# pyMSE/NLOTrajectories

Hardware: AMD Instinct MI355X
Metric: solved trajectories/sec (50-knot unicycle+learned-SDF) (higher is better)
Workload: dtype f64 (interior-point solver) + f32 (SDF-MLP: fp32-equivalent split-bf16 MFMA products, as the reference's fp32 libtorch graph)

## Files before the change

nlotrajectories_amd/csrc/nlot_solver.hip:

```cpp
#include <hip/hip_runtime.h>

#include <algorithm>
#include <chrono>
#include <type_traits>
#include <cmath>
#include <cstdlib>
#include <cstdio>
#include <cstring>
#include <vector>

#include "nlot_device.h"
#include "nlot_internal.h"
#include "nlot_solver_ws.h"

namespace nlot {

#ifndef NLOT_WPE_A
#define NLOT_WPE_A 2
#endif
#ifndef NLOT_WPE_B
#define NLOT_WPE_B 2
#endif
#ifndef NLOT_WPE_ACC
#define NLOT_WPE_ACC 3
// ... 2350 lines not shown
            const double dy = AT(X, (seg + 1) * NX + 1) - AT(X, seg * NX + 1);
            const double rr = sqrt(dx * dx + dy * dy + p.path_eps);
            const double sgn = seg == k ? -1.0 : 1.0;
            r[0] += sgn * dx / rr;
            r[1] += sgn * dy / rr;
        }
        if (k > 0)
#pragma unroll
            for (int i = 0; i < NX; ++i) r[i] += AT(yk, (k - 1) * NX + i);
        double A[NX][NX], Bu[NX][NU];
        if (k < N) {
            double x[NX], u[NU];
#pragma unroll
            for (int i = 0; i < NX; ++i) x[i] = AT(X, k * NX + i);
#pragma unroll
            for (int i = 0; i < NU; ++i) u[i] = AT(U, k * NU + i);
            Dyn<DYN>::jac(x, u, p.dt, p.wheelbase, A, Bu);
#pragma unroll
            for (int j = 0; j < NX; ++j) {
                double t = 0;
#pragma unroll
                for (int i = 0; i < NX; ++i) t += A[i][j] * AT(yk, k * NX + i);
                r[j] -= t;
            }
        }
        if (k == 0)
#pragma unroll
            for (int i = 0; i < NX; ++i) r[i] += AT(yi, i);
        if (k == N)
#pragma unroll
            for (int i = 0; i < NX; ++i)
                for (int cc = 0; cc < nc; ++cc)
                    if (dm.tidx[cc] == i) r[i] += AT(yt, cc);
        for (int j = 0; j < M; ++j)
            for (int a = 0; a < 3 && a < NX; ++a) r[a] += AT(Jd, (k * M + j) * 3 + a) * AT(yd, k * M + j);
#pragma unroll
        for (int i = 0; i < NX; ++i) {
            dual = fmax(dual, fabs(r[i]));
            dsq += r[i] * r[i];
            d1 += fabs(r[i]);
        }
        if (k < N)
#pragma unroll
            for (int i = 0; i < NU; ++i) {
                double t = dm.gcb ? AT(yb, k * NU + i) : -AT(zl, k * NU + i) + AT(zu, k * NU + i);
                if (p.use_smooth && k < N - 1) t += 2.0 * p.smooth_weight * AT(U, k * NU + i);
#pragma unroll
                for (int a = 0; a < NX; ++a) t -= Bu[a][i] * AT(yk, k * NX + a);
                dual = fmax(dual, fabs(t));
                dsq += t * t;
                d1 += fabs(t);
            }
        if (dm.ns) {
            double t = 2.0 * p.slack_penalty * AT(S, k) + (dm.gcb ? AT(yb, N * NU + k) : -AT(zs, k));
            if (dm.sd)
                for (int j = 0; j < M; ++j) t += AT(yd, k * M + j);
            dual = fmax(dual, fabs(t));
            dsq += t * t;
            d1 += fabs(t);
        }
        for (int j = 0; j < M; ++j) {
            const double t = -AT(yd, k * M + j) - AT(vt, k * M + j);
            dual = fmax(dual, fabs(t));
            dsq += t * t;
            d1 += fabs(t);
        }
    }
    p_bs.run(ngb, lane, ld_bs, [&](int q, const double* v) {
        const double t = q < nnu ? -v[0] - v[1] + v[2] : -v[0] - v[1];
        dual = fmax(dual, fabs(t));
        dsq += t * t;
        d1 += fabs(t);
    });
    auto pri_ = [&](double v) {
        primal = fmax(primal, fabs(v));
        psq += v * v;
        p1 += fabs(v);
    };
    auto pri1 = [&](int, const double* v) { pri_(v[0]); };
    p_rci.run(NX, lane, ld_rci, pri1);
    p_rct.run(nc, lane, ld_rct, pri1);
    p_rcd.run(N * NX, lane, ld_rcd, pri1);
    cviol = wmax(primal);
    p_rcq.run((N + 1) * M, lane, ld_rcq, [&](int, const double* v) {
        pri_(v[0]);
        cviol = fmax(cviol, fmax(0.0, -v[1]));
    });
    p_rcb.run(ngb, lane, ld_rcb, [&](int q, const double* v) {
        pri_(v[0]);
        if (q < nnu) {
            const double u = v[1];
            cviol = fmax(cviol, fmax(0.0, fmax(p.umin[q % NU] - u, u - p.umax[q % NU])));
        } else {
            cviol = fmax(cviol, fmax(0.0, -v[1]));
        }
    });
    auto compl_ = [&](double z, double s) {
        c0 = fmax(c0, fabs(z * s));
        cmu = fmax(cmu, fabs(z * s - mu0));
        csum += z * s;
        zsum += fabs(z);
        nzc += 1;
    };
    p_cu.run(N * NU, lane, ld_cu, [&](int e, const double* v) {
        compl_(v[1], v[0] - p.umin[e % NU]);
        compl_(v[2], p.umax[e % NU] - v[0]);
    });
    auto compl2 = [&](int, const double* v) { compl_(v[0], v[1]); };
    if (dm.ns) p_zs.run(N + 1, lane, ld_zs, compl2);
    p_vt.run((N + 1) * M, lane, ld_vt, compl2);
    auto ysum1 = [&](int, const double* v) { ysum += fabs(v[0]); };
    p_yi.run(NX, lane, ld_yi, ysum1);
    p_yk.run(N * NX, lane, ld_yk, ysum1);
    p_yt.run(nc, lane, ld_yt, ysum1);
    p_yd.run((N + 1) * M, lane, ld_yd, ysum1);
    p_yb.run(ngb, lane, ld_yb, ysum1);
    dual = wmax(dual);
    primal = wmax(primal);
    cviol = wmax(cviol);
    c0 = wmax(c0);
    cmu = wmax(cmu);
    zsum = wsum(zsum);
    ysum = wsum(ysum);
    nzc = wsum(nzc);
    const double csum_w = wsum(csum), dsq_w = wsum(dsq), psq_w = wsum(psq);
    const double d1_w = wsum(d1), p1_w = wsum(p1);
    const double ny = NX + N * NX + nc + (N + 1) * M + ngb;
    const double sd = fmax(100.0, (ysum + zsum) / (ny + nzc)) / 100.0;
    const double scc = fmax(100.0, zsum / nzc) / 100.0;
    const double E0 = fmax(fmax(dual / sd, primal), c0 / scc);
    KPROF(0, 3);
    const double n_pd = (double)((N + 1) * NX + N * NU + dm.ns * (N + 1) + (N + 1) * M + ngb) +
                        (double)(NX + nc + N * NX + (N + 1) * M + ngb) + nzc;
    auto pd_error = [&](double m) {
        double c1 = 0;
        for (int e = lane; e < N * NU; e += 64) {
            const double u = BVU(e);
            c1 += fabs(AT(zl, e) * (u - p.umin[e % NU]) - m) + fabs(AT(zu, e) * (p.umax[e % NU] - u) - m);
        }
        if (dm.ns)
            for (int k = lane; k <= N; k += 64) c1 += fabs(AT(zs, k) * BVS(k) - m);
        for (int q = lane; q < (N + 1) * M; q += 64) c1 += fabs(AT(vt, q) * AT(T, q) - m);
        return (d1_w + p1_w + wsum(c1)) / n_pd;
    };
    if (ph == PH_SOFT2) {
        const double pd_t = pd_error(SC(SC_MUPD));
        const bool ok = isfinite(pd_t) && pd_t <= o.soft_resto_pderror_reduction_factor * SC(SC_PDC);
        wsync();
        if (!ok) {
            double* buf = &AT(sts, 0);
            iter_io(ws, b, lane, buf, false);
            wsync();
            resto_enter(o, p, dm, ws, b, lane, cnt_next);
            return;
        }
        if (lane == 0) {
            SC(SC_ITERS) = SC(SC_ITERS) + 1;
            SC(SC_INSOFT) = 1;
            SC(SC_TINYLAST) = 0;
            SC(SC_PHASE) = PH_EVAL;
        }
        wsync();
    }
    const int iters = (int)SC(SC_ITERS);
    wsync();
    auto finish = [&](int status) {
        if (lane == 0) {
            SC(SC_E0) = E0;
            SC(SC_STATUS) = status;
            SC(SC_PHASE) = PH_DONE;
        }
    };
    if (!isfinite(E0)) return finish(NLOT_NUMERIC);
    if (E0 <= o.tol && dual <= o.dual_inf_tol && cviol <= o.constr_viol_tol && c0 <= o.compl_inf_tol)
        return finish(NLOT_SOLVED);
    if (iters >= o.max_iter) return finish(NLOT_MAXITER);
    const double kap = o.barrier_tol_factor;
    const double mu_floor = fmin(o.tol, o.compl_inf_tol) / (kap + 1.0);
    constexpr double kMuMin = 1e-11;
    double mu = mu0, tau = SC(SC_TAU);
    bool reset_filter = false;
    auto compl_mu = [&](double m) {
        double cm = 0;
        chunked_update<4, 3>(N * NU, lane, [&](int e, double* v) { v[0] = BVU(e); v[1] = AT(zl, e); v[2] = AT(zu, e); },
                             [&](int e, const double* v) {
                                 cm = fmax(cm, fabs(v[1] * (v[0] - p.umin[e % NU]) - m));
                                 cm = fmax(cm, fabs(v[2] * (p.umax[e % NU] - v[0]) - m));
                             });
        auto cm2 = [&](int, const double* v) { cm = fmax(cm, fabs(v[0] * v[1] - m)); };
        if (dm.ns) chunked_update<4, 2>(N + 1, lane, [&](int k, double* v) { v[0] = AT(zs, k); v[1] = BVS(k); }, cm2);
        chunked_update<4, 2>((N + 1) * M, lane, [&](int q, double* v) { v[0] = AT(vt, q); v[1] = AT(T, q); }, cm2);
        return wmax(cm);
    };
    bool tiny_last = o.mu_strategy == 0 && SC(SC_TINYLAST) != 0.0;
    auto barrier_decrease = [&](double cm) {
        for (;;) {
            const double Emu = fmax(fmax(dual / sd, primal), cm / scc);
            if (Emu > kap * mu && !tiny_last) break;
            tiny_last = false;
            const double nm = fmax(fmin(0.2 * mu, pow(mu, 1.5)), mu_floor);
            if (nm >= mu) break;
            mu = nm;
            tau = fmax(0.99, 1.0 - mu);
            reset_filter = true;
            cm = compl_mu(mu);
        }
    };
    bool use_qf = false;
    const double avg = csum_w / nzc;
    if (o.mu_strategy == 0) {
        if (iters > 0) barrier_decrease(cmu);
    } else {
        double mu_max = SC(SC_MUMAX);
        bool free_ = SC(SC_FREE) != 0.0;
        int naf = (int)SC(SC_NAF);
        if (iters == 0) {
            mu_max = 1e3 * avg;
            free_ = true;
            naf = 0;
        }
        double th_c, ph_c, f_c;
        theta_phi(mu0, &th_c, &ph_c, &f_c);
        auto af_ok = [&]() {
            const double m = 1e-5 * fmin(1.0, th_c);
            bool bad = false;
            for (int i = lane; i < naf; i += 64)
                if (f_c + m >= AT(afilt, 2 * i) && th_c + m >= AT(afilt, 2 * i + 1)) bad = true;
            return __ballot(bad) == 0ull;
        };
        if (!free_) {
            if (af_ok()) {
                free_ = true;
            } else if (fmax(fmax(dual / sd, primal), cmu / scc) <= kap * mu) {
                const double nm = fmax(fmin(0.2 * mu, pow(mu, 1.5)), mu_floor);
                if (nm < mu) {
                    mu = nm;
                    tau = fmax(0.99, 1.0 - mu);
                    reset_filter = true;
                }
            }
        }
        int naf_new = naf;
        if (free_) {
            if (af_ok()) {
                const double m = 1e-5 * fmin(1.0, th_c), nf = f_c - m, nt = th_c - m;
                wsync();
                if (lane == 0) SC(SC_NAF) = naf;
                wsync();
                naf_new = filter_update(ws, b, &AT(afilt, 0), SC_NAF, nf, nt, cnt, lane);
            } else {
                free_ = false;
                mu = fmin(fmax(0.8 * avg, kMuMin), mu_max);
                tau = fmax(0.99, 1.0 - mu);
                reset_filter = true;
            }
        }
        if (lane == 0) {
            SC(SC_NAF) = naf_new;
            SC(SC_FREE) = free_ ? 1.0 : 0.0;
            SC(SC_MUMAX) = mu_max;
        }
        use_qf = free_;
    }
    const double mu_pd = (o.mu_strategy == 1 && use_qf) ? 0.0 : mu;
    const double pd_c = pd_error(mu_pd);
    wsync();
    if (lane == 0) {
        SC(SC_MU) = mu;
        SC(SC_TAU) = tau;
        if (reset_filter) {
            SC(SC_NFILT) = 0;
            SC(SC_INSOFT) = 0;
            SC(SC_SOFTCNT) = 0;
            SC(SC_WD) = 0;
            SC(SC_WDSHORT) = 0;
        }
        SC(SC_PDC) = pd_c;
        SC(SC_MUPD) = mu_pd;
    }
    wsync();
    KPROF(0, 4);
    SV::template build_stages<false>(p, dm, ws, b, lane, MODE_NEWTON, 0.0, use_qf ? 0.0 : mu, avg, use_qf ? 2 : 1, SL);
    KPROF(0, 5);
    KPROF_COUNT(0);
    if (lane == 0) {
        SC(SC_E0) = E0;
        SC(SC_RMU0) = use_qf ? 0.0 : mu;
        SC(SC_RMU1) = avg;
        SC(SC_RNR) = use_qf ? 2 : 1;
        SC(SC_USEQF) = use_qf ? 1.0 : 0.0;
        SC(SC_AVG) = avg;
        SC(SC_DSQ) = dsq_w;
        SC(SC_PSQ) = psq_w;
        SC(SC_NZC) = nzc;
        SC(SC_PRIMAL) = primal;
        SC(SC_RICFIX) = -1.0;
        SC(SC_RIC) = 1;
        ws.ricl[atomicAdd(&cnt[4], 1)] = b;
    }
}

template <int DYN>
__global__ __launch_bounds__(64) __attribute__((amdgpu_waves_per_eu(NLOT_WPE_B))) void k_iter_b(const NlotProblem* __restrict__ pp_, const Dims* __restrict__ dd_, NlotSolverOptions o, const Ws* __restrict__ ws_,
                                               const int* __restrict__ active, int* cnt, float* tp, int* cnt_next) {
    grid_guard(*ws_, cnt[2], 1, GRID_ACTIVE);
    if ((int)blockIdx.x >= cnt[2]) return;
    const NlotProblem& p = *pp_;
    const Dims& dm = *dd_;
    const Ws& ws = *ws_;
    using SV = Solver<DYN>;
    constexpr int NX = SV::NX, NU = SV::NU;
    const int b = active[blockIdx.x], lane = threadIdx.x;
    if (SC(SC_RESTO) != 0.0) return;
    const int ric = (int)SC(SC_RIC);
    if (ric == 4) {
        double* rb = &AT(rcs, 0);
        double* sb = &AT(sts, 0);
        {
            double* buf = rb;
            const bool save = false;
            res_io(ws, b, lane, buf, save);
            buf = sb;
            step_io(ws, b, lane, buf, save);
        }
        const double na = 0.5 * SC(SC_SOCA);
        const bool failed = na < SC(SC_AMIN);
        wsync();
        if (lane == 0) {
            SC(SC_RIC) = 0;
            SC(SC_SOCK) = 0;
            SC(SC_AZ) = SC(SC_SOCAZ);
            SC(SC_TRIALS) = 1;
            SC(SC_ALPHA) = na;
            if (!failed) SC(SC_PHASE) = PH_LS;
        }
        wsync();
        if (failed) ls_failed(o, *pp_, *dd_, ws, b, lane, tp, cnt, cnt_next);
        else emit_points(*pp_, *dd_, ws, b, lane, cnt, true, tp, 1, na);
        return;
    }
    if (ric != 2) return;
    KPROF_INIT;
    const bool soc = (int)SC(SC_PHASE) == PH_SOC;
    const int N = dm.N, M = dm.M;
    const double dw = SC(SC_DW), avg = SC(SC_AVG), dsq_w = SC(SC_DSQ), psq_w = SC(SC_PSQ), nzc = SC(SC_NZC);
    const bool use_qf = SC(SC_USEQF) != 0.0;
    double mu = SC(SC_MU), tau = SC(SC_TAU);
    const int ngb = dm.gcb ? dm.ngb : 0;
    const int n_dual_ = (N + 1) * NX + N * NU + dm.ns * (N + 1) + (N + 1) * M + ngb;
    const int n_pri_ = NX + dm.nc + N * NX + (N + 1) * M + ngb;
    const int nc = dm.nc;
    constexpr double kMuMin = 1e-11;
    (void)o;
    auto theta_phi = [&](double mu, double* th, double* phv, double* fout = nullptr) {
        double t = 0, bar = 0, lin = 0;
        auto tsum = [&](int, const double* v) { t += fabs(v[0]); };
        auto l_rci = [&](int i, double* v) { v[0] = AT(rci, i); };
        auto l_rct = [&](int i, double* v) { v[0] = AT(rct, i); };
        auto l_rcd = [&](int i, double* v) { v[0] = AT(rcd, i); };
        auto l_rcq = [&](int q, double* v) { v[0] = AT(rcq, q); v[1] = AT(T, q); };
        auto l_bu = [&](int e, double* v) { v[0] = BVU(e); };
        auto l_bs = [&](int k, double* v) { v[0] = BVS(k); };
        auto l_rcb = [&](int q, double* v) { v[0] = AT(rcb, q); };
        Pre<1, 1> q_rci, q_rct, q_bs;
        Pre<4, 1> q_rcd;
        Pre<1, 2> q_rcq;
        Pre<2, 1> q_bu;
        Pre<3, 1> q_rcb;
        q_rci.load(NX, lane, l_rci);
        q_rct.load(nc, lane, l_rct);
        q_rcd.load(N * NX, lane, l_rcd);
        q_rcq.load((N + 1) * M, lane, l_rcq);
        q_bu.load(N * NU, lane, l_bu);
        if (dm.ns) q_bs.load(N + 1, lane, l_bs);
        q_rcb.load(ngb, lane, l_rcb);
        q_rci.run(NX, lane, l_rci, tsum);
        q_rct.run(nc, lane, l_rct, tsum);
        q_rcd.run(N * NX, lane, l_rcd, tsum);
        q_rcq.run((N + 1) * M, lane, l_rcq, [&](int, const double* v) {
            t += fabs(v[0]);
            bar += log(v[1]);
            lin += v[1];
        });
        q_bu.run(N * NU, lane, l_bu, [&](int e, const double* v) {
            const double u = v[0];
            bar += log(u - p.umin[e % NU]) + log(p.umax[e % NU] - u);
        });
        if (dm.ns)
            q_bs.run(N + 1, lane, l_bs, [&](int, const double* v) {
                bar += log(v[0]);
                lin += v[0];
            });
        q_rcb.run(ngb, lane, l_rcb, tsum);
        *th = wsum(t);
        const double fo = objective_w(p, dm, ws, b, lane, 0.0);
        *phv = fo - mu * wsum(bar) + 1e-5 * mu * wsum(lin);
        if (fout) *fout = fo;
    };
    {
        const int oU = (N + 1) * NX, oS = oU + N * NU, oyi = oS + N + 1, oyk = oyi + NX, oyt = oyk + N * NX,
                  oT = oyt + 8, ozl = oT + (N + 1) * M, ozu = ozl + N * NU, ozs = ozu + N * NU, ovt = ozs + N + 1,
                  odb = ovt + (N + 1) * M;
        const int oBU = dm.gcb ? odb : oU, oBS = dm.gcb ? odb + N * NU : oS;
        auto qf_store = [&](double m, bool cen) {
            double* dst = cen ? &AT(qc, 0) : &AT(qa, 0);
            const double* aff = &AT(qa, 0);
            const double* sX = cen ? &AT(dX2, 0) : &AT(dX, 0);
            const double* sU = cen ? &AT(dU2, 0) : &AT(dU, 0);
            const double* sS = cen ? &AT(dS2, 0) : &AT(dS, 0);
            const double* syi = cen ? &AT(yi2, 0) : &AT(yi_n, 0);
            const double* syk = cen ? &AT(yk2, 0) : &AT(yk_n, 0);
            const double* syt = cen ? &AT(yt2, 0) : &AT(yt_n, 0);
            auto put = [&](int i, double v) { dst[i] = cen ? v - aff[i] : v; };
            for (int i = lane; i < (N + 1) * NX; i += 64) put(i, sX[i]);
            for (int i = lane; i < N * NU; i += 64) put(oU + i, sU[i]);
            for (int i = lane; i <= N; i += 64) put(oS + i, sS[i]);
            for (int i = lane; i < NX; i += 64) put(oyi + i, syi[i]);
            for (int i = lane; i < N * NX; i += 64) put(oyk + i, syk[i]);
            for (int i = lane; i < 8; i += 64) put(oyt + i, syt[i]);
            for (int k = lane; k <= N; k += 64) {
                for (int j = 0; j < M; ++j) {
                    const int q = k * M + j;
                    double Jdz = 0;
                    for (int a = 0; a < 3 && a < NX; ++a) Jdz += AT(Jd, q * 3 + a) * sX[k * NX + a];
                    if (dm.sd) Jdz += sS[k];
                    const double t = AT(T, q), v = AT(vt, q), dt_ = Jdz + AT(rcq, q);
                    put(oT + q, dt_);
                    put(ovt + q, m / t - v - (v / t) * dt_);
                }
                if (dm.ns) {
                    const double sk = BVS(k), ds = dm.gcb ? sS[k] + AT(rcb, N * NU + k) : sS[k];
                    put(ozs + k, m / sk - AT(zs, k) - (AT(zs, k) / sk) * ds);
                    if (dm.gcb) put(odb + N * NU + k, ds);
                }
            }
            for (int e = lane; e < N * NU; e += 64) {
                const double u = BVU(e), sl = u - p.umin[e % NU], su = p.umax[e % NU] - u;
                const double du = dm.gcb ? sU[e] + AT(rcb, e) : sU[e];
                put(ozl + e, m / sl - AT(zl, e) - (AT(zl, e) / sl) * du);
                put(ozu + e, m / su - AT(zu, e) + (AT(zu, e) / su) * du);
                if (dm.gcb) put(odb + e, du);
            }
            wsync();
        };
        if (use_qf) {
        qf_store(0.0, false);
        qf_store(avg, true);
        const double* qa_ = &AT(qa, 0);
        const double* qc_ = &AT(qc, 0);
        const double dual_t = dsq_w / (double)n_dual_, pri_t = psq_w / (double)n_pri_;
        const bool qf_fast = N * NU <= 128 && N + 1 <= 64 && (N + 1) * M <= 64;
        constexpr int QP = 6;
        double c_sl[QP], c_isl[QP], c_da[QP], c_dc[QP], c_z[QP], c_iz[QP], c_za[QP], c_zc[QP];
        if (qf_fast) {
            auto put = [&](int j, double sl, double da, double dc, double z, double za, double zc) {
                c_sl[j] = sl;
                c_isl[j] = 1.0 / sl;
                c_da[j] = da;
                c_dc[j] = dc;
                c_z[j] = z;
                c_iz[j] = 1.0 / z;
                c_za[j] = za;
                c_zc[j] = zc;
            };
            auto none = [&](int j) {
                c_sl[j] = 1.0; c_isl[j] = 0.0; c_da[j] = c_dc[j] = 0.0;
                c_z[j] = 0.0; c_iz[j] = 0.0; c_za[j] = c_zc[j] = 0.0;
            };
#pragma unroll
            for (int h = 0; h < 2; ++h) {
                const int e = lane + 64 * h;
                if (e < N * NU) {
                    const double u = BVU(e), da = qa_[oBU + e], dc = qc_[oBU + e];
                    put(2 * h, u - p.umin[e % NU], da, dc, AT(zl, e), qa_[ozl + e], qc_[ozl + e]);
                    put(2 * h + 1, p.umax[e % NU] - u, -da, -dc, AT(zu, e), qa_[ozu + e], qc_[ozu + e]);
                } else {
                    none(2 * h);
                    none(2 * h + 1);
                }
            }
            if (dm.ns && lane <= N) put(4, BVS(lane), qa_[oBS + lane], qc_[oBS + lane], AT(zs, lane), qa_[ozs + lane],
                                        qc_[ozs + lane]);
            else none(4);
            if (lane < (N + 1) * M) put(5, AT(T, lane), qa_[oT + lane], qc_[oT + lane], AT(vt, lane), qa_[ovt + lane],
                                        qc_[ovt + lane]);
            else none(5);
        }
        auto qf = [&](double sig) {
            const double tq = fmax(0.99, 1.0 - sig * avg);
            if (qf_fast) {
                double rp = 0.0, rd = 0.0;
#pragma unroll
                for (int j = 0; j < QP; ++j) {
                    rp = fmax(rp, -(c_da[j] + sig * c_dc[j]) * c_isl[j]);
                    rd = fmax(rd, -(c_za[j] + sig * c_zc[j]) * c_iz[j]);
                }
                rp = wmax(rp);
                rd = wmax(rd);
                const double ap = rp > 0.0 ? fmin(1.0, tq / rp) : 1.0, ad = rd > 0.0 ? fmin(1.0, tq / rd) : 1.0;
                double csq = 0.0;
#pragma unroll
                for (int j = 0; j < QP; ++j) {
                    const double c = (c_sl[j] + ap * (c_da[j] + sig * c_dc[j])) * (c_z[j] + ad * (c_za[j] + sig * c_zc[j]));
                    csq += c * c;
                }
                csq = wsum(csq);
                return (1.0 - ad) * (1.0 - ad) * dual_t + (1.0 - ap) * (1.0 - ap) * pri_t + csq / nzc;
            }
            double ap = 1.0, ad = 1.0;
            for (int e = lane; e < N * NU; e += 64) {
                const double u = BVU(e), du = qa_[oBU + e] + sig * qc_[oBU + e];
                ap = frac_to_bound(u - p.umin[e % NU], du, tq, ap);
                ap = frac_to_bound(p.umax[e % NU] - u, -du, tq, ap);
                ad = frac_to_bound(AT(zl, e), qa_[ozl + e] + sig * qc_[ozl + e], tq, ad);
                ad = frac_to_bound(AT(zu, e), qa_[ozu + e] + sig * qc_[ozu + e], tq, ad);
            }
            if (dm.ns)
                for (int k = lane; k <= N; k += 64) {
                    ap = frac_to_bound(BVS(k), qa_[oBS + k] + sig * qc_[oBS + k], tq, ap);
                    ad = frac_to_bound(AT(zs, k), qa_[ozs + k] + sig * qc_[ozs + k], tq, ad);
                }
            for (int q = lane; q < (N + 1) * M; q += 64) {
                ap = frac_to_bound(AT(T, q), qa_[oT + q] + sig * qc_[oT + q], tq, ap);
                ad = frac_to_bound(AT(vt, q), qa_[ovt + q] + sig * qc_[ovt + q], tq, ad);
            }
            ap = wmin(ap);
            ad = wmin(ad);
            double csq = 0;
            auto cq = [&](double sl, double dsl, double z, double dz) {
                const double c = (sl + ap * dsl) * (z + ad * dz);
                csq += c * c;
            };
            for (int e = lane; e < N * NU; e += 64) {
                const double u = BVU(e), du = qa_[oBU + e] + sig * qc_[oBU + e];
                cq(u - p.umin[e % NU], du, AT(zl, e), qa_[ozl + e] + sig * qc_[ozl + e]);
                cq(p.umax[e % NU] - u, -du, AT(zu, e), qa_[ozu + e] + sig * qc_[ozu + e]);
            }
            if (dm.ns)
                for (int k = lane; k <= N; k += 64)
                    cq(BVS(k), qa_[oBS + k] + sig * qc_[oBS + k], AT(zs, k), qa_[ozs + k] + sig * qc_[ozs + k]);
            for (int q = lane; q < (N + 1) * M; q += 64)
                cq(AT(T, q), qa_[oT + q] + sig * qc_[oT + q], AT(vt, q), qa_[ovt + q] + sig * qc_[ovt + q]);
            csq = wsum(csq);
            return (1.0 - ad) * (1.0 - ad) * dual_t + (1.0 - ap) * (1.0 - ap) * pri_t + csq / nzc;
        };
        const double mu_max = SC(SC_MUMAX);
        const double sig_up = fmin(100.0, mu_max / avg), sig_lo = fmax(1e-6, kMuMin / avg);
        const double gfac = (3.0 - sqrt(5.0)) / 2.0;
        enum { EV_1M, EV_1, EV_M1, EV_M2, EV_N1, EV_N2, EV_UP, EV_LO, LOOP, FINAL, DONE };
        bool lg = false;
        double tu0 = 0, tl0 = 0, up = 0, lo = 0, m1 = 0, m2 = 0, q1 = 0, q2 = 0, q_up = -1, q_lo = -1, q1m = 0,
               qq = 0, sig = sig_up;
        int nsec = 0, st;
        auto toS = [&](double t_) { return lg ? pow(10.0, t_) : t_; };
        auto start = [&](double su, double qu, double sl, double ql, bool l) {
            lg = l;
            tu0 = up = lg ? log10(su) : su;
            tl0 = lo = lg ? log10(sl) : sl;
            q_up = qu;
            q_lo = ql;
            m1 = lo + gfac * (up - lo);
            m2 = lo + (1.0 - gfac) * (up - lo);
            nsec = 0;
        };
        if (sig_lo >= sig_up) {
            st = DONE;
        } else if (sig_up <= 1.0) {
            start(sig_up, -1.0, sig_lo, -1.0, true);
            st = EV_M1;
        } else if (sig_lo >= 1.0) {
            start(sig_up, -1.0, sig_lo, -1.0, false);
            st = EV_M1;
        } else {
            st = EV_1M;
        }
        while (st != DONE) {
            const double x = st == EV_1M ? 0.99
                           : st == EV_1  ? 1.0
                           : (st == EV_M1 || st == EV_N1) ? toS(m1)
                           : (st == EV_M2 || st == EV_N2) ? toS(m2)
                           : st == EV_UP ? toS(up)
                                         : toS(lo);
            const double qv = qf(x);
            switch (st) {
                case EV_1M: q1m = qv; st = EV_1; break;
                case EV_1:
                    if (q1m > qv) start(sig_up, -1.0, 1.0, qv, false);
                    else start(0.99, q1m, sig_lo, -1.0, true);
                    st = EV_M1;
                    break;
                case EV_M1: q1 = qv; st = EV_M2; break;
                case EV_M2: q2 = qv; st = LOOP; break;
                case EV_N1: q1 = qv; st = LOOP; break;
                case EV_N2: q2 = qv; st = LOOP; break;
                case EV_UP: q_up = qv; st = FINAL; break;
                default: q_lo = qv; st = FINAL; break;
            }
            while (st == LOOP || st == FINAL) {
                if (st == LOOP) {
                    if (nsec < 8 && (toS(up) - toS(lo)) >= 1e-2 * toS(up)) {
                        ++nsec;
                        if (q1 > q2) {
                            lo = m1; q_lo = q1; m1 = m2; q1 = q2;
                            m2 = lo + (1.0 - gfac) * (up - lo);
                            st = EV_N2;
                        } else {
                            up = m2; q_up = q2; m2 = m1; q2 = q1;
                            m1 = lo + gfac * (up - lo);
                            st = EV_N1;
                        }
                    } else {
                        sig = q1 < q2 ? toS(m1) : toS(m2);
                        qq = q1 < q2 ? q1 : q2;
                        if (up == tu0) st = q_up < 0 ? EV_UP : FINAL;
                        else if (lo == tl0) st = q_lo < 0 ? EV_LO : FINAL;
// ... 1498 lines not shown
```

nlotrajectories_amd/csrc/nlot_solver_run.h:

```cpp
#pragma once
#include <algorithm>
#include <chrono>
#include <cstdio>
#include <cstdlib>
#include <cstring>
#include <vector>

#include "nlot_solver_ws.h"

namespace nlot {

extern thread_local NlotSolveStats g_stats;
extern int g_timing;

#define NLOT_RC_CHECK(expr)                              \
    do {                                                 \
        if (const int rc_ = (expr)) return rc_;          \
    } while (0)

constexpr int KPIPE = 8;

struct RunKnobs {
    int setprio = 0;
    int stream_prio = 0;
    int soc_fork = 0;
    bool early_value = true;
    bool mlp_reuse = true;
    int spec_threshold = 8192;
    int spec_bulk = 2;
    int ric_tries = 1;
    int ric_tries_min = 0;
    bool resto_tries = true;
    double progress_s = 0;
    int kpipe = KPIPE;
    int resto_force = 0;
    bool step_kernel = true;
    const char* step_log = nullptr;
};

static RunKnobs read_knobs(const MlpDev* w, int64_t P) {
    RunKnobs k;
    if (w) {
        const double H = w->H, fwd = 2.0 * (2.0 * H + w->n_hidden * H * H + H);
        k.spec_threshold = (int)std::max(1.0, std::min(1e9, 5.6e10 / (fwd * (double)P)));
    }
    if (const char* e = getenv("NLOT_SETPRIO")) k.setprio = atoi(e);
    if (const char* e = getenv("NLOT_STREAM_PRIO")) k.stream_prio = atoi(e);
    if (const char* e = getenv("NLOT_SOC_FORK")) k.soc_fork = std::max(0, std::min(2, atoi(e)));
    if (const char* e = getenv("NLOT_EARLY_VALUE")) k.early_value = atoi(e) != 0;
    if (const char* e = getenv("NLOT_MLP_REUSE")) k.mlp_reuse = strcmp(e, "0") != 0;
    if (const char* e = getenv("NLOT_SPEC_THRESHOLD")) k.spec_threshold = atoi(e);
    if (const char* e = getenv("NLOT_SPEC_BULK")) k.spec_bulk = std::max(1, std::min(NSPEC, atoi(e)));
    if (const char* e = getenv("NLOT_RIC_TRIES")) k.ric_tries = std::max(1, atoi(e));
    if (const char* e = getenv("NLOT_RIC_TRIES_MIN")) k.ric_tries_min = atoi(e);
    if (const char* e = getenv("NLOT_RESTO_TRIES")) k.resto_tries = atoi(e) != 0;
    if (const char* e = getenv("NLOT_PROGRESS")) k.progress_s = atof(e);
    if (const char* e = getenv("NLOT_PIPE")) k.kpipe = std::max(1, std::min(KPIPE, atoi(e)));
    if (const char* e = getenv("NLOT_RESTO_BOUND")) k.resto_force = std::max(1, atoi(e));
    if (const char* e = getenv("NLOT_STEP_KERNEL")) k.step_kernel = atoi(e) != 0;
    k.step_log = getenv("NLOT_STEP_LOG");
    return k;
}

struct Res {
    int* hcnt = nullptr;
    int* dcnt = nullptr;
    hipEvent_t ev[KPIPE][10] = {};
    hipEvent_t noev[10] = {};
    bool timed[KPIPE] = {};
    hipStream_t s2 = nullptr, s3 = nullptr, s4 = nullptr;
    hipEvent_t e_a = nullptr, e_soc = nullptr, e_r = nullptr, e_s = nullptr, e_v0 = nullptr, e_v1 = nullptr;
    int create(int stream_prio, bool timing) {
        NLOT_HIP_CHECK(hipHostMalloc((void**)&hcnt, (KPIPE * 2 * CSET + 2) * sizeof(int),
                                     hipHostMallocMapped | hipHostMallocCoherent));
        if (stream_prio > 0) {
            int prio_least = 0, prio_greatest = 0;
            NLOT_HIP_CHECK(hipDeviceGetStreamPriorityRange(&prio_least, &prio_greatest));
            if (stream_prio >= 2) NLOT_HIP_CHECK(hipStreamCreateWithPriority(&s2, hipStreamNonBlocking, prio_greatest));
            else NLOT_HIP_CHECK(hipStreamCreateWithFlags(&s2, hipStreamNonBlocking));
            NLOT_HIP_CHECK(hipStreamCreateWithPriority(&s3, hipStreamNonBlocking, prio_greatest));
        } else {
            NLOT_HIP_CHECK(hipStreamCreateWithFlags(&s2, hipStreamNonBlocking));
            NLOT_HIP_CHECK(hipStreamCreateWithFlags(&s3, hipStreamNonBlocking));
        }
        for (hipEvent_t* e : {&e_a, &e_soc, &e_r, &e_s, &e_v0, &e_v1})
            NLOT_HIP_CHECK(hipEventCreateWithFlags(e, hipEventDisableTiming));
        NLOT_HIP_CHECK(hipStreamCreateWithFlags(&s4, hipStreamNonBlocking));
        if (timing)
            for (auto& r : ev)
                for (auto& e : r) NLOT_HIP_CHECK(hipEventCreate(&e));
        return NLOT_OK;
    }
    ~Res() {
        for (auto& r : ev)
            for (auto& e : r)
                if (e) (void)hipEventDestroy(e);
        for (hipEvent_t e : {e_a, e_soc, e_r, e_s, e_v0, e_v1})
            if (e) (void)hipEventDestroy(e);
        if (s2) (void)hipStreamDestroy(s2);
        if (s3) (void)hipStreamDestroy(s3);
        if (s4) (void)hipStreamDestroy(s4);
        if (hcnt) (void)hipHostFree(hcnt);
    }
};

struct RunCtx {
    const NlotSolverOptions& o;
    const NlotMlp* mlp;
    hipStream_t st;
    RunKnobs kn;
    bool use_mlp = false;
    int64_t P = 0;
    int Bi = 0, capacity = 0, t_every = 0;
    Ws ws{};
    NlotProblem* dP = nullptr;
    Dims* dD = nullptr;
    Ws* dW = nullptr;
    Res res;
    MlpOut mo{}, mo_t[2] = {};
    MlpReuse reuse[2] = {};
    int64_t step = 0, synced = 0;
    int n_active = 0, cur = 0;
    bool init_step = true;
    int next_admit = 0;
    int resto_bound = 0;
    std::vector<int> slog;

    template <int DYN>
    int launch_step();
    int sync_window();
    void fold(int64_t last);
    int admit(const double* x0, const double* xg, const double* Xinit);
};

inline void RunCtx::fold(int64_t last) {
    for (int64_t sj = synced; sj <= last; ++sj) {
        const int j = (int)(sj % kn.kpipe), qj = (int)(sj & 1);
        const int* hc = res.hcnt + 2 * CSET * j + CSET * qj;
        const int next_active = res.hcnt[2 * CSET * j + CSET * (qj ^ 1) + 2];
        if (kn.step_log) {
            slog.push_back((int)sj);
            slog.push_back(n_active);
            for (int i = 0; i < 8; ++i) slog.push_back(i == 2 ? 0 : hc[i]);
            slog.push_back(next_active);
            for (int i = 8; i < 11; ++i) slog.push_back(hc[i]);
            slog.push_back(hc[15]);
        }
        g_stats.iterations = (int)(sj + 1);
        if (use_mlp) {
            g_stats.mlp_points_full += (int64_t)hc[0] * P;
            g_stats.mlp_points_value += (int64_t)hc[1] * P;
            g_stats.mlp_points_full_reused += (int64_t)hc[3];
            g_stats.mlp_full_launches++;
            g_stats.mlp_value_launches++;
        }
        g_stats.ric_launches++;
        g_stats.ric_solves += hc[4];
        g_stats.ric_soc_solves += hc[6];
        g_stats.ric_resto_solves += hc[7];
        g_stats.filter_peak = std::max(g_stats.filter_peak, hc[11]);
        g_stats.filter_forgotten += hc[12];
        const hipEvent_t* e = res.ev[j];
        if (res.timed[j]) {
            g_stats.timed_steps++;
            g_stats.timed_ric_solves += hc[4];
            if (use_mlp) {
                g_stats.timed_points_full += (int64_t)hc[0] * P;
                g_stats.timed_points_value += (int64_t)hc[1] * P;
                g_stats.timed_points_full_reused += (int64_t)hc[3];
            }
        }
        if (res.timed[j] && use_mlp) {
            float a = 0, v = 0;
            (void)hipEventElapsedTime(&a, e[0], e[1]);
            (void)hipEventElapsedTime(&v, e[2], e[3]);
            g_stats.mlp_full_ms += a;
            g_stats.mlp_value_ms += v;
            if (kn.early_value) {
                float v0 = 0;
                (void)hipEventElapsedTime(&v0, e[8], e[9]);
                g_stats.mlp_value_ms += v0;
            }
        }
        if (res.timed[j]) {
            float a = 0, r = 0;
            (void)hipEventElapsedTime(&a, e[4], e[5]);
            (void)hipEventElapsedTime(&r, e[6], e[7]);
            g_stats.iterate_ms += a;
            g_stats.ric_ms += r;
        }
        n_active = next_active;
        if (n_active == 0) break;
    }
    synced = last + 1;
}

template <int DYN>
int RunCtx::launch_step() {
    const hipStream_t s2 = res.s2, s3 = res.s3, s4 = res.s4;
    const int ric_blocks_per = RicG<DYN>::IPW;
    const int* act = ws.act[cur];
    int* nxt = ws.act[cur ^ 1];
    const int* actr = ws.actr[cur];
    int* nxtr = ws.actr[cur ^ 1];
    const int kq = (int)(step % kn.kpipe);
    res.timed[kq] = t_every > 0 && step % t_every == (step / t_every) % t_every;
    hipEvent_t* ev = res.timed[kq] ? res.ev[kq] : res.noev;
    const int q = (int)(step & 1);
    int* C = ws.cnt + CSET * q;
    int* Cn = ws.cnt + CSET * (q ^ 1);
    if (!kn.step_kernel) NLOT_HIP_CHECK(hipMemsetAsync(Cn, 0, CSET * sizeof(int), st));
    auto launch_ric = [&](const int* list, const int* count, int mode, int* diag, int tries) {
        hipLaunchKernelGGL((k_ric<DYN, false>), dim3((n_active + ric_blocks_per - 1) / ric_blocks_per), dim3(64), 0,
                           st, dP, dD, dW, list, n_active, count, mode, diag, tries);
    };
    auto soc_chain = [&](bool with_pass) {
        NLOT_HIP_CHECK(hipEventRecord(res.e_s, st));
        NLOT_HIP_CHECK(hipStreamWaitEvent(s2, res.e_s, 0));
        if (with_pass)
            hipLaunchKernelGGL(k_iter_a<DYN>, dim3(n_active), dim3(64), 0, s2, dP, dD, o, dW, act, ws.x0s, ws.xgs,
                               (int)PASS_SOC, C, Cn);
        hipLaunchKernelGGL((k_ric<DYN, false, true>), dim3((n_active + ric_blocks_per - 1) / ric_blocks_per),
                           dim3(64), 0, s2, dP, dD, dW, ws.socl, n_active, C + 6, (int)MODE_NEWTON, nullptr, 1 << 30);
        NLOT_HIP_CHECK(hipEventRecord(res.e_soc, s2));
        return NLOT_OK;
    };
    if (kn.soc_fork == 1) NLOT_RC_CHECK(soc_chain(true));
    if (use_mlp && kn.early_value) {
        if (!kn.step_kernel) NLOT_HIP_CHECK(hipMemcpyAsync(C + 14, C + 1, sizeof(int), hipMemcpyDeviceToDevice, st));
        NLOT_HIP_CHECK(hipEventRecord(res.e_v0, st));
        NLOT_HIP_CHECK(hipStreamWaitEvent(s4, res.e_v0, 0));
        if (ev[0]) (void)hipEventRecord(ev[8], s4);
        const int rc = launch_mlp_strided(mlp->dev, ws.tpts[q], (int64_t)n_active * NSPEC, C + 14, (int)P, 0, nullptr,
                                          mo_t[q], false, s4);
        if (ev[0]) (void)hipEventRecord(ev[9], s4);
        NLOT_RC_CHECK(rc);
        NLOT_HIP_CHECK(hipEventRecord(res.e_v1, s4));
    }
    const int nspec = n_active > kn.spec_threshold ? kn.spec_bulk : NSPEC;
    if (use_mlp) {
        if (init_step) hipLaunchKernelGGL(k_points, dim3(n_active), dim3(64), 0, st, dP, dD, dW, act, C);
        if (ev[0]) (void)hipEventRecord(ev[0], st);
        MlpReuse ru = reuse[q ^ 1];
        ru.nreused = C + 3;
        NLOT_RC_CHECK(launch_mlp_strided(mlp->dev, ws.pts, n_active, C + 0, (int)P, 0, nullptr, mo, true, st, &ru));
        if (ev[0]) (void)hipEventRecord(ev[1], st);
    }
    if (kn.soc_fork == 2) NLOT_RC_CHECK(soc_chain(true));
    if (ev[4]) (void)hipEventRecord(ev[4], st);
    const int n_resto = std::min(n_active, resto_bound);
    if (n_resto > 0) {
        NLOT_HIP_CHECK(hipEventRecord(res.e_a, st));
        NLOT_HIP_CHECK(hipStreamWaitEvent(s3, res.e_a, 0));
        hipLaunchKernelGGL(k_resto_a<DYN>, dim3(n_resto), dim3(64), 0, s3, dP, dD, o, dW, actr, ws.x0s, ws.xgs, C);
        hipLaunchKernelGGL((k_ric<DYN, true>), dim3((n_resto + ric_blocks_per - 1) / ric_blocks_per), dim3(64), 0, s3,
                           dP, dD, dW, actr, n_resto, C + 5, (int)MODE_NEWTON, C + 15,
                           kn.resto_tries && n_active > kn.ric_tries_min ? kn.ric_tries : 1 << 30);
        hipLaunchKernelGGL(k_resto_b<DYN>, dim3(n_resto), dim3(64), 0, s3, dP, dD, o, dW, actr, C,
                           use_mlp ? ws.tpts[q] : nullptr);
        NLOT_HIP_CHECK(hipEventRecord(res.e_r, s3));
    }
    if (init_step) {
        hipLaunchKernelGGL(k_iter_a<DYN>, dim3(n_active), dim3(64), 0, st, dP, dD, o, dW, act, ws.x0s, ws.xgs,
                           (int)PASS_INIT, C, Cn);
        launch_ric(act, C + 2, (int)MODE_LSQ, nullptr, 1 << 30);
    }
    hipLaunchKernelGGL(k_iter_a<DYN>, dim3(n_active), dim3(64), 0, st, dP, dD, o, dW, act, ws.x0s, ws.xgs,
                       (int)(kn.soc_fork == 0 ? PASS_ALL : PASS_EVAL), C, Cn);
    if (kn.soc_fork == 0) NLOT_RC_CHECK(soc_chain(false));
    if (ev[6]) (void)hipEventRecord(ev[6], st);
    launch_ric(ws.ricl, C + 4, (int)MODE_NEWTON, C + 8, n_active > kn.ric_tries_min ? kn.ric_tries : 1 << 30);
    if (ev[6]) (void)hipEventRecord(ev[7], st);
    NLOT_HIP_CHECK(hipStreamWaitEvent(st, res.e_soc, 0));
    hipLaunchKernelGGL(k_iter_b<DYN>, dim3(n_active), dim3(64), 0, st, dP, dD, o, dW, act, C,
                       use_mlp ? ws.tpts[q] : nullptr, Cn);
    if (n_resto > 0) NLOT_HIP_CHECK(hipStreamWaitEvent(st, res.e_r, 0));
    if (ev[4]) (void)hipEventRecord(ev[5], st);
    if (use_mlp) {
        if (kn.early_value) NLOT_HIP_CHECK(hipStreamWaitEvent(st, res.e_v1, 0));
        if (ev[0]) (void)hipEventRecord(ev[2], st);
        MlpReuse vb{};
        vb.base = C + 14;
        NLOT_RC_CHECK(launch_mlp_strided(mlp->dev, ws.tpts[q], (int64_t)n_active * NSPEC, C + 1, (int)P, 0, nullptr,
                                         mo_t[q], false, st, kn.early_value ? &vb : nullptr));
        if (ev[0]) (void)hipEventRecord(ev[3], st);
    }
    if (n_resto > 0)
        hipLaunchKernelGGL(k_resto_ls<DYN>, dim3(n_resto), dim3(64), 0, st, dP, dD, o, dW, actr, ws.x0s, ws.xgs, C, Cn,
                           use_mlp ? ws.tpts[q ^ 1] : nullptr, use_mlp ? ws.tval[q] : nullptr, nspec);
    hipLaunchKernelGGL(k_accept<DYN>, dim3(n_active), dim3(64), 0, st, dP, dD, o, dW, act, nxt, nxtr, ws.x0s, ws.xgs, C, Cn,
                       use_mlp ? ws.tpts[q ^ 1] : nullptr, use_mlp ? ws.tval[q] : nullptr, nspec);
    NLOT_HIP_CHECK(hipGetLastError());
    if (kn.step_kernel) {
        hipLaunchKernelGGL(k_step_end, dim3(1), dim3(64), 0, st, ws.cnt, q, res.dcnt + 2 * CSET * kq,
                           res.dcnt + KPIPE * 2 * CSET);
    } else {
        NLOT_HIP_CHECK(hipMemcpyAsync(res.hcnt + 2 * CSET * kq, ws.cnt, 2 * CSET * sizeof(int),
                                      hipMemcpyDeviceToHost, st));
    }
    cur ^= 1;
    init_step = false;
    return NLOT_OK;
}

inline int RunCtx::sync_window() {
    int* hflag = res.hcnt + KPIPE * 2 * CSET;
    if (!kn.step_kernel)
        NLOT_HIP_CHECK(hipMemcpyAsync(hflag, ws.cnt + 2 * CSET, 2 * sizeof(int), hipMemcpyDeviceToHost, st));
    NLOT_HIP_CHECK(hipStreamSynchronize(st));
    if (hflag[1] != 0) {
        set_error(grid_error(hflag[1]));
        return NLOT_ERR_INVALID;
    }
    const int kq = (int)(step % kn.kpipe);
    int rmax = 0;
    for (int j = 0; j <= kq; ++j) rmax = std::max(rmax, res.hcnt[2 * CSET * j + CSET * (((step - kq + j) & 1) ^ 1) + 5]);
    resto_bound = std::min(Bi, 2 * rmax + 256);
    if (kn.resto_force) resto_bound = std::min(resto_bound, kn.resto_force);
    fold(step);
    return NLOT_OK;
}

inline int RunCtx::admit(const double* x0, const double* xg, const double* Xinit) {
    if (next_admit >= Bi || (capacity - n_active < std::max(1, capacity / 32) && n_active != 0))
        return NLOT_OK;
    const int n_new = std::min(capacity - n_active, Bi - next_admit);
    int* Cadm = ws.cnt + CSET * ((step + 1) & 1);
    hipLaunchKernelGGL(k_admit, dim3(1), dim3(1024), 0, st, ws.act[cur], Cadm, ws.sinst, ws.freel,
                       ws.cnt + 2 * CSET, next_admit, n_new);
    hipLaunchKernelGGL(k_init_state, dim3(n_new), dim3(64), 0, st, dP, dD, o, ws, x0, xg, Xinit, ws.act[cur],
                       Cadm);
    NLOT_HIP_CHECK(hipGetLastError());
    next_admit += n_new;
    n_active += n_new;
    init_step = true;
    return NLOT_OK;
}

static int dump_kprof(hipStream_t st) {
#ifdef NLOT_KPROF
    unsigned long long kp[4][16];
    NLOT_HIP_CHECK(hipStreamSynchronize(st));
    NLOT_HIP_CHECK(hipMemcpyFromSymbol(kp, HIP_SYMBOL(g_kprof), sizeof(kp)));
    const char* kn[4] = {"k_iter_a", "k_iter_b", "k_accept", "k_resto"};
    for (int k = 0; k < 4; ++k)
        if (kp[k][15]) {
            fprintf(stderr, "[kprof] %s waves %llu: us per wave", kn[k], kp[k][15]);
            for (int i = 0; i < 15; ++i)
                if (kp[k][i]) fprintf(stderr, " [%d] %.2f", i, kp[k][i] * 1e-2 / kp[k][15]);
            fprintf(stderr, "\n");
        }
    const unsigned long long z[4][16] = {};
    NLOT_HIP_CHECK(hipMemcpyToSymbol(HIP_SYMBOL(g_kprof), z, sizeof(z)));
#endif
    return NLOT_OK;
}
static int dump_ric_prof(hipStream_t st) {
#ifdef NLOT_RIC_PROF
    unsigned long long hp[3][5];
    NLOT_HIP_CHECK(hipStreamSynchronize(st));
    NLOT_HIP_CHECK(hipMemcpyFromSymbol(hp, HIP_SYMBOL(g_ric_prof), sizeof(hp)));
    const char* kinds[3] = {"newton", "correction", "restoration"};
    for (int k = 0; k < 3; ++k)
        if (hp[k][4])
            fprintf(stderr, "[ric_prof] %s solves %llu: us per solve backward %.2f F1 %.2f F2 %.2f F3+mult %.2f\n",
                    kinds[k], hp[k][4], hp[k][0] * 1e-2 / hp[k][4], hp[k][1] * 1e-2 / hp[k][4],
                    hp[k][2] * 1e-2 / hp[k][4], hp[k][3] * 1e-2 / hp[k][4]);
    const unsigned long long z[3][5] = {};
    NLOT_HIP_CHECK(hipMemcpyToSymbol(HIP_SYMBOL(g_ric_prof), z, sizeof(z)));
#endif
    return NLOT_OK;
}

static void write_step_log(const char* path, const std::vector<int>& slog) {
    if (!path || slog.empty()) return;
    if (FILE* f = fopen(path, "a")) {
        for (size_t i = 0; i < slog.size(); i += 15) {
            for (int j = 0; j < 15; ++j) fprintf(f, j ? " %d" : "%d", slog[i + j]);
            fputc('\n', f);
        }
        fclose(f);
    }
}

template <int DYN>
int run(const NlotProblem& p, const NlotSolverOptions& o, const NlotMlp* mlp, const double* x0, const double* xg,
        const double* Xinit, double* X, double* U, double* S, double* cost, int32_t* status, int32_t* iters,
        int64_t B, void* workspace, hipStream_t st) {
    Dims dm = make_dims(p);
    dm.gcb = o.general_bounds ? 1 : 0;
    const bool use_mlp = p.sdf_kind == NLOT_SDF_MLP;
    const int64_t P = (int64_t)dm.ppk * (dm.N + 1);
    const int cap_slots = (int)slot_count(B, o.max_active);
    RunCtx c{o, mlp, st, read_knobs(use_mlp ? &mlp->dev : nullptr, P)};
    const RunKnobs& kn = c.kn;
    c.use_mlp = use_mlp;
    c.P = P;
    c.Bi = (int)B;
    c.capacity = c.next_admit = c.n_active = cap_slots;
    Ws& ws = c.ws;
    ws = carve(dm, cap_slots, use_mlp, workspace);
    ws.oX = X;
    ws.oU = U;
    ws.oS = S;
    ws.ocost = cost;
    ws.ostat = status;
    ws.oiters = iters;
    ws.prio = kn.setprio;
    c.dP = (NlotProblem*)((char*)workspace + kHdrProblem);
    c.dD = (Dims*)((char*)workspace + kHdrDims);
    c.dW = (Ws*)((char*)workspace + kHdrWs);
    static_assert(sizeof(NlotProblem) <= kHdrDims - kHdrProblem && sizeof(Dims) <= kHdrWs - kHdrDims &&
                  sizeof(Ws) <= kHdr - kHdrWs, "workspace header");
    NLOT_HIP_CHECK(hipMemcpyAsync(c.dP, &p, sizeof(NlotProblem), hipMemcpyHostToDevice, st));
    NLOT_HIP_CHECK(hipMemcpyAsync(c.dD, &dm, sizeof(Dims), hipMemcpyHostToDevice, st));
    NLOT_HIP_CHECK(hipMemcpyAsync(c.dW, &ws, sizeof(Ws), hipMemcpyHostToDevice, st));
    g_stats = NlotSolveStats{};
    g_stats.filter_capacity = FILT_MAX;
    g_stats.timing_every = c.t_every = g_timing;
    g_stats.slots_in_lds = 0;
    hipLaunchKernelGGL(k_init_state, dim3(cap_slots), dim3(64), 0, st, c.dP, c.dD, o, ws, x0, xg, Xinit, nullptr, nullptr);
    NLOT_HIP_CHECK(hipGetLastError());
    Res& res = c.res;
    NLOT_RC_CHECK(res.create(kn.stream_prio, c.t_every != 0));
    if (use_mlp) {
        const int64_t plane = P * (int64_t)cap_slots * NSPEC;
        MlpOut& mo = c.mo;
        mo.val = ws.mo; mo.gx = ws.mo + plane; mo.gy = ws.mo + 2 * plane; mo.hxx = ws.mo + 3 * plane;
        mo.hxy = ws.mo + 4 * plane; mo.hyx = mo.hxy; mo.hyy = ws.mo + 5 * plane;
        mo.sv = mo.sg = mo.sh = 1;
        for (int q = 0; q < 2; ++q) {
            c.mo_t[q].val = ws.tval[q];
            c.mo_t[q].sv = 1;
            c.mo_t[q].mask = ws.tmask[q];
            c.mo_t[q].mask_plane = plane;
            c.reuse[q] = MlpReuse{kn.mlp_reuse ? ws.tsrc : nullptr, ws.tpts[q], ws.tval[q], ws.tmask[q], plane, nullptr};
        }
    }
    const auto t0 = std::chrono::steady_clock::now();
    double t_prog = kn.progress_s;
    const int64_t waves = (B + cap_slots - 1) / cap_slots;
    const int64_t max_steps = ((int64_t)o.max_iter + 2) * 64 * (waves + 1);
    c.resto_bound = o.resto ? (kn.resto_force ? std::min(c.Bi, kn.resto_force) : c.Bi) : 0;
    NLOT_HIP_CHECK(hipMemsetAsync(ws.cnt, 0, 64 * sizeof(int), st));
    res.hcnt[0] = cap_slots;
    NLOT_HIP_CHECK(hipMemcpyAsync(ws.cnt + 2, res.hcnt, sizeof(int), hipMemcpyHostToDevice, st));
    NLOT_HIP_CHECK(hipStreamSynchronize(st));
    NLOT_HIP_CHECK(hipHostGetDevicePointer((void**)&res.dcnt, res.hcnt, 0));
    for (c.step = 0; c.step < max_steps && c.n_active > 0; ++c.step) {
        NLOT_RC_CHECK(c.launch_step<DYN>());
        if (c.step % kn.kpipe != kn.kpipe - 1) continue;
        NLOT_RC_CHECK(c.sync_window());
        if (kn.progress_s > 0) {
            const double t = std::chrono::duration<double>(std::chrono::steady_clock::now() - t0).count();
            if (t >= t_prog) {
                fprintf(stderr, "[nlot] %.0f s: step %lld, %d active, %d of %d instances admitted\n", t,
                        (long long)c.step, c.n_active, c.next_admit, c.Bi);
                fflush(stderr);
                t_prog = t + kn.progress_s;
            }
        }
        NLOT_RC_CHECK(c.admit(x0, xg, Xinit));
    }
    if (c.synced < c.step) {
        NLOT_HIP_CHECK(hipStreamSynchronize(st));
        c.fold(c.step - 1);
    }
    NLOT_RC_CHECK(dump_kprof(st));
    NLOT_RC_CHECK(dump_ric_prof(st));
    if (c.n_active > 0 || c.next_admit < c.Bi) {
        set_error("nlot_solve_batch: the global step cap was reached with instances unfinished (phase-machine bug)");
        return NLOT_ERR_INVALID;
    }
    write_step_log(kn.step_log, c.slog);
    NLOT_HIP_CHECK(hipMemcpyAsync(res.hcnt, ws.cnt + 2 * CSET, 2 * sizeof(int), hipMemcpyDeviceToHost, st));
    NLOT_HIP_CHECK(hipStreamSynchronize(st));
    if (res.hcnt[1] != 0 || res.hcnt[0] != cap_slots) {
        set_error(res.hcnt[1] != 0 ? grid_error(res.hcnt[1])
                                   : "nlot_solve_batch: slot bookkeeping mismatch (free slots at the end != capacity)");
        return NLOT_ERR_INVALID;
    }
    return NLOT_OK;
}

}
```

Before: 1685.

## Split iter_b into per-list launches overlapping SOC and Newton streams

k_iter_b now takes an explicit list and count, so it can run once over the Newton Riccati list on the main stream and once over the SOC list on the side stream. Previously it waited for the SOC chain and then ran over all active problems. The aim is to let the SOC tail overlap with main-stream work and remove the join before iter_b. The cost is an extra launch and a changed grid_guard class (GRID_SOLVE), and correctness now depends on the ricl and socl lists together covering every problem that needs iter_b.

```diff
diff --git a/nlotrajectories_amd/csrc/nlot_solver.hip b/nlotrajectories_amd/csrc/nlot_solver.hip
--- a/nlotrajectories_amd/csrc/nlot_solver.hip
+++ b/nlotrajectories_amd/csrc/nlot_solver.hip
@@ -2676,15 +2676,17 @@
 
 template <int DYN>
 __global__ __launch_bounds__(64) __attribute__((amdgpu_waves_per_eu(NLOT_WPE_B))) void k_iter_b(const NlotProblem* __restrict__ pp_, const Dims* __restrict__ dd_, NlotSolverOptions o, const Ws* __restrict__ ws_,
-                                               const int* __restrict__ active, int* cnt, float* tp, int* cnt_next) {
-    grid_guard(*ws_, cnt[2], 1, GRID_ACTIVE);
-    if ((int)blockIdx.x >= cnt[2]) return;
+                                               const int* __restrict__ list, const int* __restrict__ count, int* cnt,
+                                               float* tp, int* cnt_next) {
+    const int nlist = *count;
+    grid_guard(*ws_, nlist, 1, GRID_SOLVE);
+    if ((int)blockIdx.x >= nlist) return;
     const NlotProblem& p = *pp_;
     const Dims& dm = *dd_;
     const Ws& ws = *ws_;
     using SV = Solver<DYN>;
     constexpr int NX = SV::NX, NU = SV::NU;
-    const int b = active[blockIdx.x], lane = threadIdx.x;
+    const int b = list[blockIdx.x], lane = threadIdx.x;
     if (SC(SC_RESTO) != 0.0) return;
     const int ric = (int)SC(SC_RIC);
     if (ric == 4) {
diff --git a/nlotrajectories_amd/csrc/nlot_solver_run.h b/nlotrajectories_amd/csrc/nlot_solver_run.h
--- a/nlotrajectories_amd/csrc/nlot_solver_run.h
+++ b/nlotrajectories_amd/csrc/nlot_solver_run.h
@@ -36,6 +36,7 @@
     int resto_force = 0;
     bool step_kernel = true;
     const char* step_log = nullptr;
+    bool iterb_split = true;
 };
 
 static RunKnobs read_knobs(const MlpDev* w, int64_t P) {
@@ -59,6 +60,7 @@
     if (const char* e = getenv("NLOT_RESTO_BOUND")) k.resto_force = std::max(1, atoi(e));
     if (const char* e = getenv("NLOT_STEP_KERNEL")) k.step_kernel = atoi(e) != 0;
     k.step_log = getenv("NLOT_STEP_LOG");
+    if (const char* e = getenv("NLOT_ITERB_SPLIT")) k.iterb_split = atoi(e) != 0;
     return k;
 }
 
@@ -214,6 +216,19 @@
         hipLaunchKernelGGL((k_ric<DYN, false>), dim3((n_active + ric_blocks_per - 1) / ric_blocks_per), dim3(64), 0,
                            st, dP, dD, dW, list, n_active, count, mode, diag, tries);
     };
+    auto iter_b = [&](const int* list, const int* count, hipStream_t s) {
+        hipLaunchKernelGGL(k_iter_b<DYN>, dim3(n_active), dim3(64), 0, s, dP, dD, o, dW, list, count, C,
+                           use_mlp ? ws.tpts[q] : nullptr, Cn);
+    };
+    auto soc_tail = [&](bool after_mlp) {
+        if (after_mlp) {
+            NLOT_HIP_CHECK(hipEventRecord(res.e_s, st));
+            NLOT_HIP_CHECK(hipStreamWaitEvent(s2, res.e_s, 0));
+        }
+        if (kn.iterb_split) iter_b(ws.socl, C + 6, s2);
+        NLOT_HIP_CHECK(hipEventRecord(res.e_soc, s2));
+        return NLOT_OK;
+    };
     auto soc_chain = [&](bool with_pass) {
         NLOT_HIP_CHECK(hipEventRecord(res.e_s, st));
         NLOT_HIP_CHECK(hipStreamWaitEvent(s2, res.e_s, 0));
@@ -222,8 +237,7 @@
                                (int)PASS_SOC, C, Cn);
         hipLaunchKernelGGL((k_ric<DYN, false, true>), dim3((n_active + ric_blocks_per - 1) / ric_blocks_per),
                            dim3(64), 0, s2, dP, dD, dW, ws.socl, n_active, C + 6, (int)MODE_NEWTON, nullptr, 1 << 30);
-        NLOT_HIP_CHECK(hipEventRecord(res.e_soc, s2));
-        return NLOT_OK;
+        return kn.soc_fork == 1 ? NLOT_OK : soc_tail(false);
     };
     if (kn.soc_fork == 1) NLOT_RC_CHECK(soc_chain(true));
     if (use_mlp && kn.early_value) {
@@ -246,6 +260,7 @@
         NLOT_RC_CHECK(launch_mlp_strided(mlp->dev, ws.pts, n_active, C + 0, (int)P, 0, nullptr, mo, true, st, &ru));
         if (ev[0]) (void)hipEventRecord(ev[1], st);
     }
+    if (kn.soc_fork == 1) NLOT_RC_CHECK(soc_tail(use_mlp && kn.iterb_split));
     if (kn.soc_fork == 2) NLOT_RC_CHECK(soc_chain(true));
     if (ev[4]) (void)hipEventRecord(ev[4], st);
     const int n_resto = std::min(n_active, resto_bound);
@@ -271,9 +286,13 @@
     if (ev[6]) (void)hipEventRecord(ev[6], st);
     launch_ric(ws.ricl, C + 4, (int)MODE_NEWTON, C + 8, n_active > kn.ric_tries_min ? kn.ric_tries : 1 << 30);
     if (ev[6]) (void)hipEventRecord(ev[7], st);
-    NLOT_HIP_CHECK(hipStreamWaitEvent(st, res.e_soc, 0));
-    hipLaunchKernelGGL(k_iter_b<DYN>, dim3(n_active), dim3(64), 0, st, dP, dD, o, dW, act, C,
-                       use_mlp ? ws.tpts[q] : nullptr, Cn);
+    if (kn.iterb_split) {
+        iter_b(ws.ricl, C + 4, st);
+        NLOT_HIP_CHECK(hipStreamWaitEvent(st, res.e_soc, 0));
+    } else {
+        NLOT_HIP_CHECK(hipStreamWaitEvent(st, res.e_soc, 0));
+        iter_b(act, C + 2, st);
+    }
     if (n_resto > 0) NLOT_HIP_CHECK(hipStreamWaitEvent(st, res.e_r, 0));
     if (ev[4]) (void)hipEventRecord(ev[5], st);
     if (use_mlp) {
```

Measured after the change: 1704, median of 6. 1.01x the previous value.
